# fudan-zvg/PARTNER

Hardware: AMD Instinct MI355X
Metric: frames/sec polar voxelize+PFN+BEV+head, 30k-pt sweep (whole job) (higher is better)
Workload: dtype f32

## Files before the change

### partner_amd/csrc/conv_wchain.hip

```cpp
#include "pn_common.h"
#include "wino_planes.h"
#include <algorithm>
#include <cstdlib>

namespace {

using f32x16 = __attribute__((ext_vector_type(16))) float;
using f32x4 = __attribute__((ext_vector_type(4))) float;
using f32x2 = __attribute__((ext_vector_type(2))) float;

struct WChainArgs {
  const float* vin;
  const float* w;
  const float* scale;
  const float* shift;
  float* vout;
  float* out;
  int B, H, W, Wq, Cin, Cout;
  int wq_log2;
  int out_ps, out_co;
  long long out_img, out_row;
  int act;
  int total_quads;
  int qtiles, ctiles;
// ... 304 lines not shown
    if (!(PN_WCHAIN_EXP & 2) || first) {
#pragma unroll
      for (int r = 0; r < 4; ++r) d[slot][r] = __builtin_bit_cast(f32x4, __builtin_amdgcn_raw_buffer_load_b128(rsrc_v, voff, so_v + (unsigned)r * row16, 0));
    }
    if (!(PN_WCHAIN_EXP & 4) || first) {
#pragma unroll
      for (int s2 = 0; s2 < 4; ++s2) u[slot][s2] = __builtin_bit_cast(f32x4, __builtin_amdgcn_raw_buffer_load_b128(rsrc_w, uoff, so_u + (unsigned)(s2 * 48) * cp16, 0));
    }
  };
  first = true;
  load_step(cg0, 0);
  __builtin_amdgcn_sched_barrier(0);
  load_step(cg0 + 1, 1);
  __builtin_amdgcn_sched_barrier(0);
  first = false;
  WC_STAMP(1);
  for (int cg = cg0; cg <= cg_last; cg += 2) {
#pragma unroll
    for (int slot = 0; slot < 2; ++slot) {
      const int nx = cg + 2 + slot <= cg_last ? cg + 2 + slot : cg_last;
      f32x4 b[4];
      if constexpr (PN_WCHAIN_EXP & 1) {
        b[0] = d[slot][0]; b[1] = d[slot][1]; b[2] = d[slot][2]; b[3] = d[slot][3];
      } else {
#pragma unroll
        for (int e = 0; e < 4; e += 2) {
          f32x2 x0 = {d[slot][0][e], d[slot][0][e + 1]}, x1 = {d[slot][1][e], d[slot][1][e + 1]}, x2 = {d[slot][2][e], d[slot][2][e + 1]},
                x3 = {d[slot][3][e], d[slot][3][e + 1]};
          f32x2 r0, r1, r2, r3;
          asm volatile("v_pk_add_f32 %0, %4, %6 neg_lo:[0,1] neg_hi:[0,1]\n\t"
                       "v_pk_add_f32 %1, %5, %6\n\t"
                       "v_pk_add_f32 %2, %6, %5 neg_lo:[0,1] neg_hi:[0,1]\n\t"
                       "v_pk_add_f32 %3, %5, %7 neg_lo:[0,1] neg_hi:[0,1]"
                       : "=&v"(r0), "=&v"(r1), "=&v"(r2), "=&v"(r3)
                       : "v"(x0), "v"(x1), "v"(x2), "v"(x3));
          b[0][e] = r0[0]; b[0][e + 1] = r0[1];
          b[1][e] = r1[0]; b[1][e + 1] = r1[1];
          b[2][e] = r2[0]; b[2][e + 1] = r2[1];
          b[3][e] = r3[0]; b[3][e + 1] = r3[1];
        }
      }
      if constexpr (PN_WCHAIN_EXP & 8) __builtin_amdgcn_s_setprio(2);
#pragma unroll
      for (int j = 0; j < 4; ++j)
#pragma unroll
        for (int s2 = 0; s2 < 4; ++s2) acc[s2] = __builtin_amdgcn_mfma_f32_32x32x2f32(u[slot][s2][j], b[s2][j], acc[s2], 0, 0, 0);
      if constexpr (PN_WCHAIN_EXP & 8) __builtin_amdgcn_s_setprio(0);
      __builtin_amdgcn_sched_barrier(0);
      load_step(nx, slot);
      __builtin_amdgcn_sched_barrier(0);
    }
  }
  WC_STAMP(2);
  if (bid != bid0) __syncthreads();
#pragma unroll
  for (int g = 0; g < 4; ++g) {
    f32x4 r0, r1;
#pragma unroll
    for (int k = 0; k < 4; ++k) {
      const int r = 4 * g + k;
      r0[k] = (acc[0][r] + acc[1][r]) + acc[2][r];
      r1[k] = (acc[1][r] - acc[2][r]) - acc[3][r];
    }
    J[((w * 2 + 0) * 4 + g) * 64 + lane] = r0;
    J[((w * 2 + 1) * 4 + g) * 64 + lane] = r1;
  }
  __syncthreads();
  for (int vw = w; vw < CT * 8; vw += NW) {
    const int ect = vw >> 3, g = (vw >> 1) & 3, row = vw & 1;
    const int c0 = (ctile * CT + ect) * 32 + 8 * g + 4 * lh;
    wchain_finish<QT>(
        a, c0, li, lh, lo,
        [&](int q, int b) {
          f32x4 m = J[(((q + 6 * (KS * (ect + CT * b))) * 2 + row) * 4 + g) * 64 + lane];
#pragma unroll
          for (int k = 1; k < KS; ++k) m += J[(((q + 6 * (k + KS * (ect + CT * b))) * 2 + row) * 4 + g) * 64 + lane];
          return m;
        },
        [&](int b, int& img, int& r, int& xq) {
          int t;
          wchain_coords(img0, t0, Hh, a.wq_log2, 32 * b + li, img, t, xq);
          r = 2 * t + row;
        },
        a.st_part ? a.st_part + ((size_t)qt * 2 + row) * a.Cout * 2 : nullptr, a.strata_rows > 0 ? ((2 * t0) / a.strata_rows) * a.Cout : 0);
  }
  WC_STAMP(3);
  }
}

template <int KS, int CT, int QT>
__global__ __launch_bounds__(64 * 6 * KS * CT * QT) void conv_wchain2_kernel(WChainArgs a) {
  wchain2_body<KS, CT, QT>(a, blockIdx.x, gridDim.x);
}

template <int SH>
__device__ __forceinline__ void wchain3_kloop(const WChainArgs& a, const __amdgpu_buffer_rsrc_t rsrc_v, const __amdgpu_buffer_rsrc_t rsrc_w, const int p,
                                              const unsigned voff, const unsigned uoff, f32x16 (&acc)[3]) {
  const unsigned cp16 = (unsigned)a.cout_pad * 16u;
  const unsigned row16 = (unsigned)a.Wq * 16u;
  f32x4 d[2][5], u[2][3];
  bool first = false;
  auto load_step = [&](int cg, int slot) __attribute__((always_inline)) {
    const unsigned so_v = (unsigned)((p * a.cg_in + cg) * 2) * a.plane_bytes + (unsigned)SH * row16;
    const unsigned so_u = (unsigned)((((cg >> 2) * 6 + 3 * SH) * 6 + p) * 8 + (cg & 3) * 2) * cp16;
    if (!(PN_WCHAIN_EXP & 2) || first) {
#pragma unroll
      for (int r = 0; r < 5; ++r) d[slot][r] = __builtin_bit_cast(f32x4, __builtin_amdgcn_raw_buffer_load_b128(rsrc_v, voff, so_v + (unsigned)r * row16, 0));
    }
    if (!(PN_WCHAIN_EXP & 4) || first) {
#pragma unroll
      for (int s2 = 0; s2 < 3; ++s2) u[slot][s2] = __builtin_bit_cast(f32x4, __builtin_amdgcn_raw_buffer_load_b128(rsrc_w, uoff, so_u + (unsigned)(s2 * 48) * cp16, 0));
    }
  };
  const int cg_last = a.cg_in - 1;
  first = true;
  load_step(0, 0);
  __builtin_amdgcn_sched_barrier(0);
  load_step(1, 1);
  __builtin_amdgcn_sched_barrier(0);
  first = false;
  for (int cg = 0; cg <= cg_last; cg += 2) {
#pragma unroll
    for (int slot = 0; slot < 2; ++slot) {
      const int nx = cg + 2 + slot <= cg_last ? cg + 2 + slot : cg_last;
      f32x4 b[3];
      const f32x4 c4 = {4.f, 4.f, 4.f, 4.f}, m4 = {-4.f, -4.f, -4.f, -4.f}, m5 = {-5.f, -5.f, -5.f, -5.f}, c2 = {2.f, 2.f, 2.f, 2.f}, m2 = {-2.f, -2.f, -2.f, -2.f};
      if constexpr (PN_WCHAIN_EXP & 1) {
        b[0] = d[slot][0]; b[1] = d[slot][1]; b[2] = d[slot][2];
      } else if constexpr (SH == 0) {
        const f32x4 e = __builtin_elementwise_fma(m4, d[slot][2], d[slot][4]), o = __builtin_elementwise_fma(m4, d[slot][1], d[slot][3]);
        b[0] = __builtin_elementwise_fma(c4, d[slot][0], __builtin_elementwise_fma(m5, d[slot][2], d[slot][4]));
        b[1] = e + o;
        b[2] = e - o;
      } else {
        const f32x4 f = d[slot][3] - d[slot][1], t = d[slot][2] - d[slot][0];
        b[0] = __builtin_elementwise_fma(c2, t, f);
        b[1] = __builtin_elementwise_fma(m2, t, f);
        b[2] = __builtin_elementwise_fma(c4, d[slot][0], __builtin_elementwise_fma(m5, d[slot][2], d[slot][4]));
      }
#pragma unroll
      for (int j = 0; j < 4; ++j)
#pragma unroll
        for (int s2 = 0; s2 < 3; ++s2) {
          if (PN_WC3_EXP & 1) acc[s2][0] += u[slot][s2][j] * b[s2][j];
          else acc[s2] = __builtin_amdgcn_mfma_f32_32x32x2f32(u[slot][s2][j], b[s2][j], acc[s2], 0, 0, 0);
        }
      __builtin_amdgcn_sched_barrier(0);
      load_step(nx, slot);
      __builtin_amdgcn_sched_barrier(0);
    }
  }
}

template <int QT>
__global__ __launch_bounds__(64 * 12) void conv_wchain3_kernel(WChainArgs a) {
  constexpr int NW = 12;
  extern __shared__ __attribute__((aligned(16))) float smem[];
  WCHAIN_FETCH_ARGS(a);
  const int tid = threadIdx.x, lane = tid & 63;
  const int w = __builtin_amdgcn_readfirstlane(tid >> 6);
  const int p = w % 6, sh = w / 6;
  const int li = lane & 31, lh = lane >> 5;
  const __amdgpu_buffer_rsrc_t rsrc_v = __builtin_amdgcn_make_buffer_rsrc(const_cast<float*>(a.vin), 0, a.vin_bytes, 0x00020000);
  const __amdgpu_buffer_rsrc_t rsrc_w = __builtin_amdgcn_make_buffer_rsrc(const_cast<float*>(a.w), 0, a.w_bytes, 0x00020000);
  const int Hq = a.H >> 2;
  f32x4* J = reinterpret_cast<f32x4*>(smem);
  f32x4* carry = J + 6 * 4 * 4 * 64;
  const float lo = a.act == PN_ACT_RELU ? 0.f : -__builtin_inff();
  const int bid = blockIdx.x;
  int qt, ctile;
  if ((a.qtiles & 7) == 0) {
    const int xcd = bid & 7, slot = bid >> 3;
    qt = xcd * (a.qtiles >> 3) + slot / a.ctiles;
    ctile = slot - (slot / a.ctiles) * a.ctiles;
  } else {
    qt = bid / a.ctiles;
    ctile = bid - qt * a.ctiles;
  }
  const int n0 = ctile * 32;
  const int o0 = qt * 32 * QT;
  const int rg0 = o0 >> a.wq_log2, img0 = rg0 / Hq, t0 = rg0 - img0 * Hq;
  const unsigned uoff = (unsigned)(((size_t)lh * a.cout_pad + n0 + li) * 16);
#pragma unroll 1
  for (int sub = 0; sub < QT; ++sub) {
    int img, t, xq;
    wchain_coords(img0, t0, Hq, a.wq_log2, 32 * sub + li, img, t, xq);
    const unsigned voff = (unsigned)(((img * (a.H + 2) + 4 * t) * a.Wq + xq) * 16) + (unsigned)lh * a.plane_bytes;
    f32x16 acc[3];
#pragma unroll
    for (int s = 0; s < 3; ++s)
#pragma unroll
      for (int r = 0; r < 16; ++r) acc[s][r] = 0.f;
    if (sh == 0) wchain3_kloop<0>(a, rsrc_v, rsrc_w, p, voff, uoff, acc);
    else wchain3_kloop<1>(a, rsrc_v, rsrc_w, p, voff, uoff, acc);
    if (PN_WC3_EXP & 2) {
      if (acc[0][0] + acc[1][3] + acc[2][7] == 1234.5f) J[lane] = f32x4{acc[0][1], acc[1][1], acc[2][1], 0.f};
    }
    if (sub > 0) __syncthreads();
    if (sh == 0 && !(PN_WC3_EXP & 2)) {
#pragma unroll
      for (int g = 0; g < 4; ++g) {
        f32x4 r0, r1, r2;
#pragma unroll
        for (int k = 0; k < 4; ++k) {
          const int r = 4 * g + k;
          r0[k] = (acc[0][r] + acc[1][r]) + acc[2][r];
          r1[k] = acc[1][r] - acc[2][r];
          r2[k] = acc[1][r] + acc[2][r];
        }
        J[((p * 4 + 0) * 4 + g) * 64 + lane] = r0;
        J[((p * 4 + 1) * 4 + g) * 64 + lane] = r1;
        J[((p * 4 + 2) * 4 + g) * 64 + lane] = r2;
        J[((p * 4 + 3) * 4 + g) * 64 + lane] = r1;
      }
    }
    __syncthreads();
    if (sh == 1 && !(PN_WC3_EXP & 2)) {
#pragma unroll
      for (int g = 0; g < 4; ++g) {
        f32x4 r0, r1, r2, r3;
#pragma unroll
        for (int k = 0; k < 4; ++k) {
          const int r = 4 * g + k;
          const float s34 = acc[0][r] + acc[1][r], d34 = acc[0][r] - acc[1][r];
          r0[k] = s34;
          r1[k] = 2.f * d34;
          r2[k] = 4.f * s34;
          r3[k] = 8.f * d34 + acc[2][r];
        }
        J[((p * 4 + 0) * 4 + g) * 64 + lane] += r0;
        J[((p * 4 + 1) * 4 + g) * 64 + lane] += r1;
        J[((p * 4 + 2) * 4 + g) * 64 + lane] += r2;
        J[((p * 4 + 3) * 4 + g) * 64 + lane] += r3;
      }
    }
    __syncthreads();
    for (int vw = w; vw < ((PN_WC3_EXP & 4) ? 0 : 16); vw += NW) {
      const int g = vw >> 2, row = vw & 3;
      const int c0 = ctile * 32 + 8 * g + 4 * lh;
      if constexpr (QT == 1) {
        wchain_finish<1>(
            a, c0, li, lh, lo, [&](int q, int) { return J[((q * 4 + row) * 4 + g) * 64 + lane]; },
            [&](int, int& im, int& r, int& x) { im = img; r = 4 * t + row; x = xq; });
      } else {
        f32x4 sc = {1.f, 1.f, 1.f, 1.f}, shf = {0.f, 0.f, 0.f, 0.f};
        if (a.scale) sc = *reinterpret_cast<const f32x4*>(a.scale + c0);
        if (a.shift) shf = *reinterpret_cast<const f32x4*>(a.shift + c0);
        f32x4 m[6], y[4];
#pragma unroll
        for (int q = 0; q < 6; ++q) m[q] = J[((q * 4 + row) * 4 + g) * 64 + lane];
        {
          const f32x4 s12 = m[1] + m[2], d12 = m[1] - m[2], s34 = m[3] + m[4], d34 = m[3] - m[4];
          const f32x4 lo4 = {lo, lo, lo, lo};
          y[0] = __builtin_elementwise_max(__builtin_elementwise_fma((m[0] + s12) + s34, sc, shf), lo4);
          y[1] = __builtin_elementwise_max(__builtin_elementwise_fma(d12 + 2.f * d34, sc, shf), lo4);
          y[2] = __builtin_elementwise_max(__builtin_elementwise_fma(s12 + 4.f * s34, sc, shf), lo4);
          y[3] = __builtin_elementwise_max(__builtin_elementwise_fma((d12 + 8.f * d34) + m[5], sc, shf), lo4);
        }
        const int r = 4 * t + row;
        if (a.out) {
          float* o = a.out + (size_t)img * a.out_img + (size_t)r * a.out_row + (size_t)(4 * xq) * a.out_ps + a.out_co + c0;
#pragma unroll
          for (int px = 0; px < 4; ++px) *reinterpret_cast<f32x4*>(o + (size_t)px * a.out_ps) = y[px];
        }
        if (a.vout) {
          f32x4* cr = carry + ((row * 4 + g) * 2 + lh) * 5;
          f32x4 l, rr;
#pragma unroll
          for (int j = 0; j < 4; ++j) {
            l[j] = __shfl_up(y[3][j], 1, 32);
            rr[j] = __shfl_down(y[0][j], 1, 32);
          }
          const f32x4 z4 = {0.f, 0.f, 0.f, 0.f};
          auto store_planes = [&](const f32x4 (&d)[6], int xs) {
            f32x4 vv[6];
            wchain_input_transform(d, vv);
            float* o = a.vout + ((size_t)(c0 >> 3) * 2 + lh) * (a.plane_bytes >> 2) + ((size_t)(img * (a.H + 2) + r + 1) * a.Wq + xs) * 4;
            const size_t pstride = (size_t)a.cg_out * 2 * (a.plane_bytes >> 2);
#pragma unroll
            for (int q = 0; q < 6; ++q) *reinterpret_cast<f32x4*>(o + q * pstride) = vv[q];
            if (r == 0) {
#pragma unroll
              for (int q = 0; q < 6; ++q) *reinterpret_cast<f32x4*>(o + q * pstride - (size_t)a.Wq * 4) = z4;
            }
            if (r == a.H - 1) {
#pragma unroll
              for (int q = 0; q < 6; ++q) *reinterpret_cast<f32x4*>(o + q * pstride + (size_t)a.Wq * 4) = z4;
            }
          };
          if (sub == 0) {
            if (li == 31) {
              cr[0] = y[0]; cr[1] = y[1]; cr[2] = y[2]; cr[3] = y[3]; cr[4] = l;
            } else {
              f32x4 d[6];
              d[0] = xq > 0 ? l : z4;
              d[1] = y[0]; d[2] = y[1]; d[3] = y[2]; d[4] = y[3];
              d[5] = rr;
              store_planes(d, xq);
            }
          } else {
            if (li == 0) {
              f32x4 d[6];
              d[0] = cr[4]; d[1] = cr[0]; d[2] = cr[1]; d[3] = cr[2]; d[4] = cr[3];
              d[5] = y[0];
              store_planes(d, xq - 1);
              l = cr[3];
            }
            f32x4 d[6];
            d[0] = l;
            d[1] = y[0]; d[2] = y[1]; d[3] = y[2]; d[4] = y[3];
            d[5] = xq + 1 < a.Wq ? rr : z4;
            store_planes(d, xq);
          }
        }
      }
    }
  }
}

__global__ void pack_wino44_weight_kernel(const float* __restrict__ w, int cout, int cin, int cout_pad, float* __restrict__ packed, size_t total) {
  for (size_t i = blockIdx.x * (size_t)blockDim.x + threadIdx.x; i < total; i += (size_t)gridDim.x * blockDim.x) {
    size_t r = i;
    const int k1 = r & 3; r >>= 2;
    const int n = (int)(r % cout_pad); r /= cout_pad;
    const int k4 = r & 7; r >>= 3;
    const int q = (int)(r % 6); r /= 6;
    const int s = (int)(r % 6);
    const int chunk = (int)(r / 6);
    const int c = chunk * 32 + k4 * 4 + k1;
    double v = 0.0;
    if (n < cout && c < cin) {
      const float* g = w + ((size_t)n * cin + c) * 9;
      auto fold = [](int pos, double g0, double g1, double g2) {
        return pos == 0 ? g0 / 4.0 : pos == 1 ? -(g0 + g1 + g2) / 6.0 : pos == 2 ? -(g0 - g1 + g2) / 6.0 : pos == 3 ? g0 / 24.0 + g1 / 12.0 + g2 / 6.0
               : pos == 4 ? g0 / 24.0 - g1 / 12.0 + g2 / 6.0 : g2;
      };
      double row[3];
      for (int kw = 0; kw < 3; ++kw) row[kw] = fold(s, g[kw], g[3 + kw], g[6 + kw]);
      v = fold(q, row[0], row[1], row[2]);
    }
    packed[i] = (float)v;
  }
}

constexpr int kChainMultiJobs = 4;
struct WChainMulti {
  int njobs;
  int first[kChainMultiJobs + 1];
  WChainArgs job[kChainMultiJobs];
};

template <int KS, int CT, int QT>
__global__ __launch_bounds__(64 * 6 * KS * CT * QT) void conv_wchain2_multi_kernel(WChainMulti by_value) {
  typedef const __attribute__((address_space(4))) int* kptr_t;
  const kptr_t base = (kptr_t)__builtin_amdgcn_kernarg_segment_ptr();
  const int njobs = base[offsetof(WChainMulti, njobs) / 4];
  const int t = blockIdx.x;
  int j = 0;
  for (int k = 1; k < njobs; ++k)
    if (t >= base[offsetof(WChainMulti, first) / 4 + k]) j = k;
  j = __builtin_amdgcn_readfirstlane(j);
  const int local = t - base[offsetof(WChainMulti, first) / 4 + j];
  constexpr int JW = sizeof(WChainArgs) / 4;
  union { WChainArgs a; int w[JW]; } u;
  const kptr_t src = base + offsetof(WChainMulti, job) / 4 + j * JW;
#pragma unroll
  for (int i = 0; i < JW; ++i) u.w[i] = src[i];
  wchain2_body<KS, CT, QT>(u.a, local, 1 << 30);
}

__global__ void pack_wino24_weight_kernel(const float* __restrict__ w, int cout, int cin, int cout_pad, float* __restrict__ packed, size_t total) {
  for (size_t i = blockIdx.x * (size_t)blockDim.x + threadIdx.x; i < total; i += (size_t)gridDim.x * blockDim.x) {
    size_t r = i;
    const int k1 = r & 3; r >>= 2;
    const int n = (int)(r % cout_pad); r /= cout_pad;
    const int k4 = r & 7; r >>= 3;
    const int q = (int)(r % 6); r /= 6;
    const int s = (int)(r & 3);
    const int chunk = (int)(r >> 2);
    const int c = chunk * 32 + k4 * 4 + k1;
    double v = 0.0;
    if (n < cout && c < cin) {
      const float* g = w + ((size_t)n * cin + c) * 9;
      double row[3];
      for (int kw = 0; kw < 3; ++kw) {
        const double g0 = g[kw], g1 = g[3 + kw], g2 = g[6 + kw];
        row[kw] = s == 0 ? g0 : s == 1 ? (g0 + g1 + g2) * 0.5 : s == 2 ? (g0 - g1 + g2) * 0.5 : g2;
      }
      const double g0 = row[0], g1 = row[1], g2 = row[2];
      v = q == 0 ? g0 / 4.0 : q == 1 ? -(g0 + g1 + g2) / 6.0 : q == 2 ? -(g0 - g1 + g2) / 6.0 : q == 3 ? g0 / 24.0 + g1 / 12.0 + g2 / 6.0
          : q == 4 ? g0 / 24.0 - g1 / 12.0 + g2 / 6.0 : g2;
    }
    packed[i] = (float)v;
  }
}

__global__ __launch_bounds__(256) void wchain_v_from_nhwc_kernel(const float* __restrict__ in, float* __restrict__ vout, int B, int H, int W, int Wq, int C,
                                                                 long long in_img, long long in_row, int in_ps, int in_co, int total_quads,
                                                                 unsigned plane_floats) {
  const int c4n = C >> 2;
  for (long long it = blockIdx.x * (long long)blockDim.x + threadIdx.x; it < (long long)total_quads * c4n; it += (long long)gridDim.x * blockDim.x) {
    const int c4 = (int)(it / total_quads);
    const int Q = (int)(it - (long long)c4 * total_quads);
    const int rowi = Q / Wq, xq = Q - rowi * Wq;
    const int img = rowi / H, r = rowi - img * H;
    const float* px = in + (size_t)img * in_img + (size_t)r * in_row + (size_t)(4 * xq) * in_ps + in_co + c4 * 4;
    f32x4 d[6], v[6];
    const f32x4 z = {0.f, 0.f, 0.f, 0.f};
    d[0] = xq > 0 ? *reinterpret_cast<const f32x4*>(px - in_ps) : z;
#pragma unroll
    for (int k = 0; k < 4; ++k) d[1 + k] = *reinterpret_cast<const f32x4*>(px + (size_t)k * in_ps);
    d[5] = xq + 1 < Wq ? *reinterpret_cast<const f32x4*>(px + (size_t)4 * in_ps) : z;
    wchain_input_transform(d, v);
    float* o = vout + (size_t)c4 * plane_floats + ((size_t)(img * (H + 2) + r + 1) * Wq + xq) * 4;
    const size_t pstride = (size_t)c4n * plane_floats;
#pragma unroll
    for (int q = 0; q < 6; ++q) *reinterpret_cast<f32x4*>(o + q * pstride) = v[q];
    if (r == 0) {
#pragma unroll
      for (int q = 0; q < 6; ++q) *reinterpret_cast<f32x4*>(o + q * pstride - (size_t)Wq * 4) = z;
    }
    if (r == H - 1) {
#pragma unroll
      for (int q = 0; q < 6; ++q) *reinterpret_cast<f32x4*>(o + q * pstride + (size_t)Wq * 4) = z;
    }
  }
}

constexpr int kHeadFinJobs = 8;
struct HeadFinJob {
  const float* part;
  int cout_total, c_off, cmid;
  int strata;
  const float* gamma;
  const float* beta;
  float eps;
  float* tab;
};
struct HeadFinArgs {
  int njobs, B, rows, tile_rows;
  long long row_pixels;
  HeadFinJob job[kHeadFinJobs];
};

__global__ __launch_bounds__(256) void wchain_head_finalize_kernel(HeadFinArgs f) {
  __shared__ double red[2][4];
  const int S0 = 8;
  const int j = blockIdx.x / (f.B * S0), rem = blockIdx.x - j * (f.B * S0), b = rem / S0, s = rem - b * S0;
  if (j >= f.njobs) return;
  const HeadFinJob& jb = f.job[j];
  const int S = jb.strata > 1 ? jb.strata : 1;
  if (s >= S) return;
  const int tid = threadIdx.x;
  const int tiles_b = f.rows / f.tile_rows;
  const float2* part = reinterpret_cast<const float2*>(jb.part);
  if (S == 1) {
    __shared__ double sl1[4][64], sl2[4][64];
    for (int c0 = 0; c0 < jb.cmid; c0 += 64) {
      const int c = c0 + (tid & 63), slice = tid >> 6;
      double a1 = 0.0, a2 = 0.0;
      if (c < jb.cmid) {
#pragma unroll 8
        for (int e = slice; e < tiles_b * 2; e += 4) {
          const float2 v = part[((size_t)b * tiles_b * 2 + e) * jb.cout_total + jb.c_off + c];
          a1 += (double)v.x;
          a2 += (double)v.y;
        }
      }
      __syncthreads();
      sl1[slice][tid & 63] = a1;
      sl2[slice][tid & 63] = a2;
      __syncthreads();
      if (tid < 64 && c < jb.cmid) {
        const double t1 = ((sl1[0][tid] + sl1[1][tid]) + sl1[2][tid]) + sl1[3][tid], t2 = ((sl2[0][tid] + sl2[1][tid]) + sl2[2][tid]) + sl2[3][tid];
        const double n = (double)f.rows * (double)f.row_pixels;
        const double mean = t1 / n;
        double var = t2 / n - mean * mean;
        var = var < 0.0 ? 0.0 : var;
        const float rstd = (float)(1.0 / sqrt(var + (double)jb.eps));
        const float ga = jb.gamma ? jb.gamma[c] : 1.f, be = jb.beta ? jb.beta[c] : 0.f;
        const float A = ga * rstd;
        reinterpret_cast<float2*>(jb.tab)[(size_t)b * jb.cmid + c] = make_float2(A, be - (float)mean * A);
      }
    }
    return;
  }
  const int tiles_s = tiles_b / S;
  const int count = tiles_s * 2 * jb.cmid;
  double t1 = 0.0, t2 = 0.0;
  for (int e = tid; e < count; e += 256) {
    const int ent = e / jb.cmid, c = e - ent * jb.cmid;
    const float2 v = part[((size_t)(b * tiles_b + s * tiles_s) * 2 + ent) * jb.cout_total + jb.c_off + c];
    t1 += (double)v.x;
    t2 += (double)v.y;
  }
  t1 = pn::wave_sum(t1);
  t2 = pn::wave_sum(t2);
  if ((tid & 63) == 0) {
    red[0][tid >> 6] = t1;
    red[1][tid >> 6] = t2;
  }
  __syncthreads();
  const double u1 = ((red[0][0] + red[0][1]) + red[0][2]) + red[0][3], u2 = ((red[1][0] + red[1][1]) + red[1][2]) + red[1][3];
  const double n = (double)(f.rows / S) * (double)f.row_pixels * jb.cmid;
  const double mean = u1 / n;
  double var = u2 / n - mean * mean;
  var = var < 0.0 ? 0.0 : var;
  const float fmean = (float)mean, rstd = (float)(1.0 / sqrt(var + (double)jb.eps));
  for (int c = tid; c < jb.cmid; c += 256) {
    const float ga = jb.gamma ? jb.gamma[s * jb.cmid + c] : 1.f, be = jb.beta ? jb.beta[s * jb.cmid + c] : 0.f;
    const float A = ga * rstd;
    reinterpret_cast<float2*>(jb.tab)[((size_t)b * S + s) * jb.cmid + c] = make_float2(A, be - fmean * A);
  }
}

static int chain_grid_limit() {
  static const int force = [] { const char* e = getenv("PN_WCHAIN_GRID"); return e ? atoi(e) : -1; }();
  if (force == 0) return 1 << 30;
  if (force > 0) return force;
  static int cus[64] = {0};
  int dev = 0;
  (void)hipGetDevice(&dev);
  if (dev < 0 || dev >= 64) return 256;
  if (cus[dev] == 0) {
    int n = 0;
    cus[dev] = (hipDeviceGetAttribute(&n, hipDeviceAttributeMultiprocessorCount, dev) == hipSuccess && n >= 8) ? n / 8 * 8 : 256;
  }
  return cus[dev];
}

struct ChainForm { int na, nb, ks, ct; };

static inline int frame_h(const pn_conv_desc* d) { return d->transpose_hw ? d->in_w : d->in_h; }
static inline int frame_w(const pn_conv_desc* d) { return d->transpose_hw ? d->in_h : d->in_w; }

static bool chain_form(const pn_conv_desc* d, ChainForm& f) {
  const int fh = frame_h(d), fw = frame_w(d);
  if (fw % 4) return false;
  const int wq = fw / 4;
  if (wq & (wq - 1)) return false;
  const long long quads = (long long)d->batch * fh * wq;
  static const int force = [] { const char* e = getenv("PN_WCHAIN_FORM"); return e ? atoi(e) : 0; }();
  const ChainForm cands[] = {{2, 2, 1, 2}, {1, 2, 2, 1}, {1, 1, 2, 1}};
  int idx = 0;
  for (const ChainForm& c : cands) {
    ++idx;
    if (force && force != idx) continue;
    const int tq = 32 * c.nb, tc = 32 * c.na * c.ct;
    if (tq % wq != 0 || quads % tq != 0 || d->cout % tc != 0 || (d->cin / 8) % c.ks != 0 || tq / wq > fh) continue;
    const long long blocks = quads / tq * (d->cout / tc);
    if (!force && blocks < 192 && idx < 3) continue;
    f = c;
    return true;
  }
  return false;
}

template <int NA, int NB, int KS, int CT>
static void launch_chain(const WChainArgs& a, hipStream_t st, bool prof, const pn::ProfileSlot& ps) {
  constexpr int NW = 6 * KS * CT;
  constexpr size_t smem = (size_t)NW * NB * 4 * 64 * 16;
  static bool done[64] = {false};
  if (pn::first_use_on_device(done))
    (void)hipFuncSetAttribute(reinterpret_cast<const void*>(&conv_wchain_kernel<NA, NB, KS, CT>), hipFuncAttributeMaxDynamicSharedMemorySize, (int)smem);
  const dim3 grid((unsigned)std::min(a.qtiles * a.ctiles, chain_grid_limit()));
  if (prof) hipExtLaunchKernelGGL((conv_wchain_kernel<NA, NB, KS, CT>), grid, dim3(64 * NW), smem, st, ps.start, ps.stop, 0, a);
  else hipLaunchKernelGGL((conv_wchain_kernel<NA, NB, KS, CT>), grid, dim3(64 * NW), smem, st, a);
}

struct Chain2Form { int ks, ct, qt; };

static bool chain2_form(const pn_conv_desc* d, Chain2Form& f, bool head = false) {
  const int fh = frame_h(d), fw = frame_w(d);
  if (fw % 4 || fh % 2) return false;
  const int wq = fw / 4;
  if (wq & (wq - 1)) return false;
  const long long octs = (long long)d->batch * (fh / 2) * wq;
  static const int prefer = [] { const char* e = getenv("PN_WCHAIN2_PREFER"); return e ? atoi(e) : 1; }();
  const bool wide_first = !head && (prefer == 2 || (prefer == 1 && d->frames_in_flight > 1)) && (octs / 64) * (d->cout / 32) >= 128;
  const Chain2Form cands_a[] = {{2, 1, 1}, {1, 1, 2}}, cands_b[] = {{1, 1, 2}, {2, 1, 1}};
  const Chain2Form* cands = wide_first ? cands_b : cands_a;
  for (int ci = 0; ci < 2; ++ci) {
    const Chain2Form& c = cands[ci];
    const int tq = 32 * c.qt, tc = 32 * c.ct;
    if (tq % wq != 0 || octs % tq != 0 || d->cout % tc != 0 || (d->cin / 8) % (2 * c.ks) != 0 || tq / wq > fh / 2) continue;
    f = c;
    return true;
  }
  return false;
}

template <int KS, int CT, int QT>
static void launch_chain2(const WChainArgs& a, hipStream_t st, bool prof, const pn::ProfileSlot& ps) {
  constexpr int NW = 6 * KS * CT * QT;
  constexpr size_t smem = (size_t)NW * 2 * 4 * 64 * 16;
  static bool done[64] = {false};
  if (pn::first_use_on_device(done))
    (void)hipFuncSetAttribute(reinterpret_cast<const void*>(&conv_wchain2_kernel<KS, CT, QT>), hipFuncAttributeMaxDynamicSharedMemorySize, (int)smem);
  const dim3 grid((unsigned)std::min(a.qtiles * a.ctiles, chain_grid_limit()));
  if (prof) hipExtLaunchKernelGGL((conv_wchain2_kernel<KS, CT, QT>), grid, dim3(64 * NW), smem, st, ps.start, ps.stop, 0, a);
  else hipLaunchKernelGGL((conv_wchain2_kernel<KS, CT, QT>), grid, dim3(64 * NW), smem, st, a);
}

template <int KS, int CT, int QT>
static void launch_chain2_multi(const WChainMulti& m, hipStream_t st, bool prof, const pn::ProfileSlot& ps) {
  constexpr int NW = 6 * KS * CT * QT;
  constexpr size_t smem = (size_t)NW * 2 * 4 * 64 * 16;
  static bool done[64] = {false};
  if (pn::first_use_on_device(done))
    (void)hipFuncSetAttribute(reinterpret_cast<const void*>(&conv_wchain2_multi_kernel<KS, CT, QT>), hipFuncAttributeMaxDynamicSharedMemorySize, (int)smem);
  const dim3 grid((unsigned)m.first[m.njobs]);
  if (prof) hipExtLaunchKernelGGL((conv_wchain2_multi_kernel<KS, CT, QT>), grid, dim3(64 * NW), smem, st, ps.start, ps.stop, 0, m);
  else hipLaunchKernelGGL((conv_wchain2_multi_kernel<KS, CT, QT>), grid, dim3(64 * NW), smem, st, m);
}

}

extern "C" {

size_t pn_wino4_planes_floats(int batch, int h, int w, int c) {
  if (batch < 1 || h < 1 || w < 4 || w % 4 || c < 8 || c % 8) return 0;
  return (size_t)6 * c * batch * (h + 2) * (w / 4);
}

static int chain_basic_ok(const pn_conv_desc* d, bool allow_strata);

int pn_conv_wino4_chain_supported(const pn_conv_desc* d) {
  if (!chain_basic_ok(d, false)) return 0;
  ChainForm f;
  return chain_form(d, f) ? 1 : 0;
}

static int chain_basic_ok(const pn_conv_desc* d, bool allow_strata) {
  if (!d) return 0;
  if (!(d->kh == 3 && d->kw == 3 && d->stride == 1 && d->pad_h == 1 && d->pad_w == 1 && d->groups == 1 && !d->deconv2x2 &&
        (d->range_strata <= 1 || allow_strata) && !d->accumulate && d->pad_h_end == 0 && d->pad_w_end == 0))
    return 0;
  if (d->batch < 1 || frame_h(d) < 1 || frame_w(d) < 4 || d->cin % 32 || d->cout % 32 || d->cin < 32) return 0;
  if (!(d->act == PN_ACT_NONE || d->act == PN_ACT_RELU)) return 0;
  if ((unsigned long long)pn_wino4_planes_floats(d->batch, frame_h(d), frame_w(d), std::max(d->cin, d->cout)) * 4ull >= (1ull << 32)) return 0;
  return 1;
}

int pn_wino4_planes_from_nhwc_f32(const float* in, int batch, int h, int w, int c, int in_pixel_stride, int in_channel_offset, int transpose_hw,
                                  float* planes, pn_stream_t stream) {
  const int stored_w = w;
  if (transpose_hw) std::swap(h, w);
  PN_REQUIRE(in && planes && pn_wino4_planes_floats(batch, h, w, c) > 0, "wino4_planes_from_nhwc: bad arguments");
  PN_REQUIRE(in_pixel_stride % 4 == 0 && in_channel_offset % 4 == 0 && in_pixel_stride >= in_channel_offset + c && ((uintptr_t)in & 15) == 0 &&
                 ((uintptr_t)planes & 15) == 0,
             "wino4_planes_from_nhwc: strides / offsets must be multiples of 4 floats, pointers 16-byte aligned");
  const int wq = w / 4;
  const long long quads = (long long)batch * h * wq;
  PN_REQUIRE(quads < (1ll << 30), "wino4_planes_from_nhwc: map too large");
  const unsigned plane_floats = (unsigned)((size_t)batch * (h + 2) * wq * 4);
  const long long items = quads * (c / 4);
  const long long in_img = (long long)h * w * in_pixel_stride;
  const long long in_row = transpose_hw ? in_pixel_stride : (long long)stored_w * in_pixel_stride;
  const int in_px = transpose_hw ? stored_w * in_pixel_stride : in_pixel_stride;
  hipLaunchKernelGGL(wchain_v_from_nhwc_kernel, dim3((unsigned)std::min<long long>(8192, (items + 255) / 256)), dim3(256), 0, pn::S(stream), in, planes, batch, h,
                     w, wq, c, in_img, in_row, in_px, in_channel_offset, (int)quads, plane_floats);
  return pn::check_launch("wchain_v_from_nhwc_kernel");
}

int pn_conv2d_wino4_chain_f32(const pn_conv_desc* d, const float* planes_in, const float* packed_w, const float* scale, const float* shift,
                              float* planes_out, float* out_nhwc, pn_stream_t stream) {
  PN_REQUIRE(d && planes_in && packed_w && (planes_out || out_nhwc), "conv_wino4_chain: null pointer");
  PN_REQUIRE(pn_conv_wino4_chain_supported(d), "conv_wino4_chain: layer shape not supported (3x3 / stride 1 / pad 1, cin and cout multiples of 32, "
                                               "row-aligned tiles)");
  PN_REQUIRE(((uintptr_t)planes_in & 15) == 0 && ((uintptr_t)packed_w & 15) == 0 && ((uintptr_t)planes_out & 15) == 0 && ((uintptr_t)out_nhwc & 15) == 0 &&
                 ((uintptr_t)scale & 15) == 0 && ((uintptr_t)shift & 15) == 0,
             "conv_wino4_chain: pointers must be 16-byte aligned");
  if (out_nhwc)
    PN_REQUIRE(d->out_pixel_stride >= d->out_channel_offset + d->cout && d->out_pixel_stride % 4 == 0 && d->out_channel_offset % 4 == 0 &&
                   (unsigned long long)d->batch * d->in_h * d->in_w * d->out_pixel_stride < (1ull << 40),
               "conv_wino4_chain: output channel slice must fit the pixel stride, in multiples of 4 floats");
  ChainForm f;
  chain_form(d, f);
  WChainArgs a{};
  a.vin = planes_in; a.w = packed_w; a.scale = scale; a.shift = shift; a.vout = planes_out; a.out = out_nhwc;
  a.B = d->batch; a.H = frame_h(d); a.W = frame_w(d); a.Wq = a.W / 4; a.Cin = d->cin; a.Cout = d->cout;
  a.out_co = d->out_channel_offset;
  a.out_img = (long long)d->in_h * d->in_w * d->out_pixel_stride;
  a.out_ps = d->transpose_hw ? d->in_w * d->out_pixel_stride : d->out_pixel_stride;
  a.out_row = d->transpose_hw ? d->out_pixel_stride : (long long)d->in_w * d->out_pixel_stride;
  a.wq_log2 = __builtin_ctz((unsigned)a.Wq);
  a.act = d->act;
  a.total_quads = d->batch * a.H * a.Wq;
  a.qtiles = a.total_quads / (32 * f.nb);
  a.ctiles = d->cout / (32 * f.na * f.ct);
  a.cg_in = d->cin / 8; a.cg_out = d->cout / 8;
  a.cout_pad = pn::cdiv(d->cout, 128) * 128;
  a.plane_bytes = (unsigned)((size_t)d->batch * (a.H + 2) * a.Wq * 16);
  a.vin_bytes = (unsigned)(pn_wino4_planes_floats(d->batch, a.H, a.W, d->cin) * 4);
  a.w_bytes = (unsigned)(pn_conv_wino4_packed_weight_floats(d->cout, d->cin) * 4);
#ifdef PN_WCHAIN_STAMP
  a.stamps = pn_wchain_stamp_buffer;
#endif
  pn::ProfileSlot ps{};
  const bool prof = pn::take_profile_slot(ps);
  hipStream_t st = pn::S(stream);
  if (f.na == 2 && f.nb == 2 && f.ks == 1 && f.ct == 2) launch_chain<2, 2, 1, 2>(a, st, prof, ps);
  else if (f.na == 1 && f.nb == 2 && f.ks == 2 && f.ct == 1) launch_chain<1, 2, 2, 1>(a, st, prof, ps);
  else launch_chain<1, 1, 2, 1>(a, st, prof, ps);
  return pn::check_launch("conv_wchain_kernel");
}

size_t pn_conv_wino24_packed_weight_floats(int cout, int cin) {
  return (size_t)pn::cdiv(cin, 32) * 4 * 6 * 8 * (size_t)(pn::cdiv(cout, 128) * 128) * 4;
}

int pn_pack_conv_weight_wino24_f32(const float* w_oihw, int cout, int cin, float* packed, pn_stream_t stream) {
  PN_REQUIRE(w_oihw && packed && cout >= 1 && cin >= 1, "pack_conv_weight_wino24: bad arguments");
  const size_t total = pn_conv_wino24_packed_weight_floats(cout, cin);
  hipLaunchKernelGGL(pack_wino24_weight_kernel, dim3((unsigned)std::min<size_t>(4096, (total + 255) / 256)), dim3(256), 0, pn::S(stream), w_oihw, cout, cin,
                     pn::cdiv(cout, 128) * 128, packed, total);
  return pn::check_launch("pack_wino24_weight_kernel");
}

static int chain2_ok(const pn_conv_desc* d, bool head, Chain2Form& f) {
  if (!chain_basic_ok(d, head) || !chain2_form(d, f, head)) return 0;
  if (d->range_strata > 1) {
    if (!d->transpose_hw || frame_h(d) % d->range_strata) return 0;
    const int rows = frame_h(d) / d->range_strata, tile_rows = 2 * (32 * f.qt) / (frame_w(d) / 4);
    if (rows % tile_rows) return 0;
  }
  return 1;
}

int pn_conv_wino24_chain_supported(const pn_conv_desc* d) {
  Chain2Form f;
  return chain2_ok(d, false, f);
}

static int chain2_fill(const pn_conv_desc* d, const float* planes_in, const float* packed_w24, const float* scale, const float* shift, float* planes_out,
                       float* out_nhwc, float* stat_partials, bool head, WChainArgs& a, Chain2Form& f) {
  PN_REQUIRE(d && planes_in && packed_w24 && (planes_out || out_nhwc), "conv_wino24_chain: null pointer");
  PN_REQUIRE(chain2_ok(d, head, f), "conv_wino24_chain: layer shape not supported (3x3 / stride 1 / pad 1, even height, cin and cout multiples of 32, "
                                    "row-pair-aligned tiles; range strata: transposed map, whole tiles per stratum)");
  PN_REQUIRE(((uintptr_t)planes_in & 15) == 0 && ((uintptr_t)packed_w24 & 15) == 0 && ((uintptr_t)planes_out & 15) == 0 && ((uintptr_t)out_nhwc & 15) == 0 &&
                 ((uintptr_t)scale & 15) == 0 && ((uintptr_t)shift & 15) == 0 && ((uintptr_t)stat_partials & 7) == 0,
             "conv_wino24_chain: pointers must be 16-byte aligned");
  PN_REQUIRE(!stat_partials || d->act == PN_ACT_NONE, "conv_wino24_chain: statistics are those of the stored output (no activation)");
  if (out_nhwc)
    PN_REQUIRE(d->out_pixel_stride >= d->out_channel_offset + d->cout && d->out_pixel_stride % 4 == 0 && d->out_channel_offset % 4 == 0,
               "conv_wino24_chain: output channel slice must fit the pixel stride, in multiples of 4 floats");
  a = WChainArgs{};
  a.vin = planes_in; a.w = packed_w24; a.scale = scale; a.shift = shift; a.vout = planes_out; a.out = out_nhwc;
  a.B = d->batch; a.H = frame_h(d); a.W = frame_w(d); a.Wq = a.W / 4; a.Cin = d->cin; a.Cout = d->cout;
  a.out_co = d->out_channel_offset;
  a.out_img = (long long)d->in_h * d->in_w * d->out_pixel_stride;
  a.out_ps = d->transpose_hw ? d->in_w * d->out_pixel_stride : d->out_pixel_stride;
  a.out_row = d->transpose_hw ? d->out_pixel_stride : (long long)d->in_w * d->out_pixel_stride;
  a.wq_log2 = __builtin_ctz((unsigned)a.Wq);
  a.act = d->act;
  a.total_quads = d->batch * a.H * a.Wq;
  a.qtiles = (a.total_quads / 2) / (32 * f.qt);
  a.ctiles = d->cout / (32 * f.ct);
  a.cg_in = d->cin / 8; a.cg_out = d->cout / 8;
  a.cout_pad = pn::cdiv(d->cout, 128) * 128;
  a.plane_bytes = (unsigned)((size_t)d->batch * (a.H + 2) * a.Wq * 16);
  a.vin_bytes = (unsigned)(pn_wino4_planes_floats(d->batch, a.H, a.W, d->cin) * 4);
  const int sets = d->range_strata > 1 ? d->range_strata : 1;
  a.w_stratum_bytes = (unsigned)(pn_conv_wino24_packed_weight_floats(d->cout, d->cin) * 4);
  a.w_bytes = a.w_stratum_bytes * (unsigned)sets;
  a.strata_rows = sets > 1 ? a.H / sets : 0;
  a.st_part = stat_partials;
#ifdef PN_WCHAIN_STAMP
  a.stamps = pn_wchain_stamp_buffer;
#endif
  return PN_OK;
}

static int chain2_run(const pn_conv_desc* d, const float* planes_in, const float* packed_w24, const float* scale, const float* shift, float* planes_out,
                      float* out_nhwc, float* stat_partials, bool head, pn_stream_t stream) {
  WChainArgs a;
  Chain2Form f;
  const int rc = chain2_fill(d, planes_in, packed_w24, scale, shift, planes_out, out_nhwc, stat_partials, head, a, f);
  if (rc != PN_OK) return rc;
  pn::ProfileSlot ps{};
  const bool prof = pn::take_profile_slot(ps);
  hipStream_t st = pn::S(stream);
  if (f.ks == 2) launch_chain2<2, 1, 1>(a, st, prof, ps);
  else launch_chain2<1, 1, 2>(a, st, prof, ps);
  return pn::check_launch("conv_wchain2_kernel");
}

int pn_conv2d_wino24_chain_f32(const pn_conv_desc* d, const float* planes_in, const float* packed_w24, const float* scale, const float* shift,
                               float* planes_out, float* out_nhwc, pn_stream_t stream) {
  return chain2_run(d, planes_in, packed_w24, scale, shift, planes_out, out_nhwc, nullptr, false, stream);
}

size_t pn_conv_wino44_packed_weight_floats(int cout, int cin) {
  return (size_t)pn::cdiv(cin, 32) * 6 * 6 * 8 * (size_t)(pn::cdiv(cout, 128) * 128) * 4;
}

int pn_pack_conv_weight_wino44_f32(const float* w_oihw, int cout, int cin, float* packed, pn_stream_t stream) {
  PN_REQUIRE(w_oihw && packed && cout >= 1 && cin >= 1, "pack_conv_weight_wino44: bad arguments");
  const size_t total = pn_conv_wino44_packed_weight_floats(cout, cin);
  hipLaunchKernelGGL(pack_wino44_weight_kernel, dim3((unsigned)std::min<size_t>(4096, (total + 255) / 256)), dim3(256), 0, pn::S(stream), w_oihw, cout, cin,
                     pn::cdiv(cout, 128) * 128, packed, total);
  return pn::check_launch("pack_wino44_weight_kernel");
}

int pn_conv_wino44_chain_supported(const pn_conv_desc* d) {
  if (!chain_basic_ok(d, false) || d->range_strata > 1) return 0;
  const int fh = frame_h(d), fw = frame_w(d);
  if (fw % 4 || fh % 4) return 0;
  const int wq = fw / 4;
  if ((wq & (wq - 1)) || wq > 64) return 0;
  const int tq = wq == 64 ? 64 : 32;
  const long long hexes = (long long)d->batch * (fh / 4) * wq;
  if (tq % wq || hexes % tq || tq / wq > fh / 4 || (d->cin / 8) % 2) return 0;
  return 1;
}

int pn_conv2d_wino44_chain_f32(const pn_conv_desc* d, const float* planes_in, const float* packed_w44, const float* scale, const float* shift,
                               float* planes_out, float* out_nhwc, pn_stream_t stream) {
  PN_REQUIRE(d && planes_in && packed_w44 && (planes_out || out_nhwc), "conv_wino44_chain: null pointer");
  PN_REQUIRE(pn_conv_wino44_chain_supported(d), "conv_wino44_chain: layer shape not supported (3x3 / stride 1 / pad 1, height a multiple of 4, at most 32 quads "
                                                "per row, cin and cout multiples of 32)");
  PN_REQUIRE(((uintptr_t)planes_in & 15) == 0 && ((uintptr_t)packed_w44 & 15) == 0 && ((uintptr_t)planes_out & 15) == 0 && ((uintptr_t)out_nhwc & 15) == 0 &&
                 ((uintptr_t)scale & 15) == 0 && ((uintptr_t)shift & 15) == 0,
             "conv_wino44_chain: pointers must be 16-byte aligned");
  if (out_nhwc)
    PN_REQUIRE(d->out_pixel_stride >= d->out_channel_offset + d->cout && d->out_pixel_stride % 4 == 0 && d->out_channel_offset % 4 == 0,
               "conv_wino44_chain: output channel slice must fit the pixel stride, in multiples of 4 floats");
  WChainArgs a{};
  a.vin = planes_in; a.w = packed_w44; a.scale = scale; a.shift = shift; a.vout = planes_out; a.out = out_nhwc;
  a.B = d->batch; a.H = frame_h(d); a.W = frame_w(d); a.Wq = a.W / 4; a.Cin = d->cin; a.Cout = d->cout;
  a.out_co = d->out_channel_offset;
  a.out_img = (long long)d->in_h * d->in_w * d->out_pixel_stride;
  a.out_ps = d->transpose_hw ? d->in_w * d->out_pixel_stride : d->out_pixel_stride;
  a.out_row = d->transpose_hw ? d->out_pixel_stride : (long long)d->in_w * d->out_pixel_stride;
  a.wq_log2 = __builtin_ctz((unsigned)a.Wq);
  a.act = d->act;
  a.total_quads = d->batch * a.H * a.Wq;
  const int qt2 = a.Wq == 64 ? 2 : 1;
  a.qtiles = (a.total_quads / 4) / (32 * qt2);
  a.ctiles = d->cout / 32;
  a.cg_in = d->cin / 8; a.cg_out = d->cout / 8;
  a.cout_pad = pn::cdiv(d->cout, 128) * 128;
  a.plane_bytes = (unsigned)((size_t)d->batch * (a.H + 2) * a.Wq * 16);
  a.vin_bytes = (unsigned)(pn_wino4_planes_floats(d->batch, a.H, a.W, d->cin) * 4);
  a.w_bytes = (unsigned)(pn_conv_wino44_packed_weight_floats(d->cout, d->cin) * 4);
#ifdef PN_WCHAIN_STAMP
  a.stamps = pn_wchain_stamp_buffer;
#endif
  constexpr size_t smem = (size_t)6 * 4 * 4 * 64 * 16 + (size_t)4 * 4 * 2 * 5 * 16;
  static bool done[64] = {false};
  if (pn::first_use_on_device(done)) {
    (void)hipFuncSetAttribute(reinterpret_cast<const void*>(&conv_wchain3_kernel<1>), hipFuncAttributeMaxDynamicSharedMemorySize, (int)smem);
    (void)hipFuncSetAttribute(reinterpret_cast<const void*>(&conv_wchain3_kernel<2>), hipFuncAttributeMaxDynamicSharedMemorySize, (int)smem);
  }
  pn::ProfileSlot ps{};
  const bool prof = pn::take_profile_slot(ps);
  const dim3 grid((unsigned)(a.qtiles * a.ctiles));
  if (qt2 == 2) {
    if (prof) hipExtLaunchKernelGGL(conv_wchain3_kernel<2>, grid, dim3(64 * 12), smem, pn::S(stream), ps.start, ps.stop, 0, a);
    else hipLaunchKernelGGL(conv_wchain3_kernel<2>, grid, dim3(64 * 12), smem, pn::S(stream), a);
  } else {
    if (prof) hipExtLaunchKernelGGL(conv_wchain3_kernel<1>, grid, dim3(64 * 12), smem, pn::S(stream), ps.start, ps.stop, 0, a);
    else hipLaunchKernelGGL(conv_wchain3_kernel<1>, grid, dim3(64 * 12), smem, pn::S(stream), a);
  }
  return pn::check_launch("conv_wchain3_kernel");
}

size_t pn_conv_wino24_chain_stat_floats(const pn_conv_desc* d) {
  Chain2Form f;
  if (!chain2_ok(d, true, f)) return 0;
  const long long octs = (long long)d->batch * (frame_h(d) / 2) * (frame_w(d) / 4);
  return (size_t)(octs / (32 * f.qt)) * 2 * d->cout * 2;
}

int pn_conv_wino24_chain_stat_tile_rows(const pn_conv_desc* d) {
  Chain2Form f;
  if (!chain2_ok(d, true, f)) return 0;
  return 2 * (32 * f.qt) / (frame_w(d) / 4);
}

int pn_conv2d_wino24_chain_head_f32(const pn_conv_desc* d, const float* planes_in, const float* packed_w24, const float* scale, const float* shift,
                                    float* planes_out, float* out_nhwc, float* stat_partials, pn_stream_t stream) {
  return chain2_run(d, planes_in, packed_w24, scale, shift, planes_out, out_nhwc, stat_partials, true, stream);
}

int pn_conv2d_wino24_chain_head_multi_f32(const pn_chain_head_job* jobs, int njobs, pn_stream_t stream) {
  PN_REQUIRE(jobs && njobs >= 1 && njobs <= kChainMultiJobs, "conv_wino24_chain_head_multi: 1 - 4 jobs");
  WChainMulti m{};
  m.njobs = njobs;
  Chain2Form f0{};
  for (int j = 0; j < njobs; ++j) {
    const pn_chain_head_job& q = jobs[j];
    Chain2Form f;
    const int rc = chain2_fill(q.desc, q.planes_in, q.packed_w24, q.scale, q.shift, q.planes_out, q.out_nhwc, q.stat_partials, true, m.job[j], f);
    if (rc != PN_OK) return rc;
    if (j == 0) f0 = f;
    PN_REQUIRE(f.ks == f0.ks && f.ct == f0.ct && f.qt == f0.qt, "conv_wino24_chain_head_multi: the jobs must share one kernel form (same map, same cin)");
    m.first[j + 1] = m.first[j] + m.job[j].qtiles * m.job[j].ctiles;
  }
  pn::ProfileSlot ps{};
  const bool prof = pn::take_profile_slot(ps);
  hipStream_t st = pn::S(stream);
  static const int ks1 = [] { const char* e = getenv("PN_WCHAIN_MULTI_KS1"); return e ? atoi(e) : 1; }();
  const bool others = ks1 == 2 || (ks1 == 1 && jobs[0].desc->frames_in_flight > 1);
  if (f0.ks == 2 && others && m.job[0].cg_in <= 8 && m.first[njobs] >= 2 * chain_grid_limit()) launch_chain2_multi<1, 1, 1>(m, st, prof, ps);
  else if (f0.ks == 2) launch_chain2_multi<2, 1, 1>(m, st, prof, ps);
  else launch_chain2_multi<1, 1, 2>(m, st, prof, ps);
  return pn::check_launch("conv_wchain2_multi_kernel");
}

int pn_wino24_chain_head_finalize_f32(const pn_head_stat_job* jobs, int njobs, int batch, int frame_rows, int frame_row_pixels, int tile_rows,
                                      pn_stream_t stream) {
  PN_REQUIRE(jobs && njobs >= 1 && njobs <= kHeadFinJobs && batch >= 1 && frame_rows >= 1 && tile_rows >= 1 && frame_rows % tile_rows == 0,
             "wino24_chain_head_finalize: bad arguments");
  HeadFinArgs f{};
  f.njobs = njobs; f.B = batch; f.rows = frame_rows; f.tile_rows = tile_rows; f.row_pixels = frame_row_pixels;
  for (int j = 0; j < njobs; ++j) {
    const pn_head_stat_job& q = jobs[j];
    PN_REQUIRE(q.partials && q.table && q.channels >= 1 && q.channel_offset >= 0 && q.channel_offset + q.channels <= q.cout_total,
               "wino24_chain_head_finalize: bad job");
    PN_REQUIRE(q.strata <= 8 && (q.strata <= 1 ? q.channels <= 256 : (frame_rows / tile_rows) % q.strata == 0),
               "wino24_chain_head_finalize: per-channel jobs take <= 256 channels; strata (<= 8) must divide the sample's tiles");
    f.job[j] = HeadFinJob{q.partials, q.cout_total, q.channel_offset, q.channels, q.strata, q.gamma, q.beta, q.eps, q.table};
  }
  hipLaunchKernelGGL(wchain_head_finalize_kernel, dim3((unsigned)(njobs * batch * 8)), dim3(256), 0, pn::S(stream), f);
  return pn::check_launch("wchain_head_finalize_kernel");
}

}
```

Before: 1766.

## Compute two output-channel tiles per block in wino44 chain conv to reuse input

Adds a two-column variant of the Winograd 4x4 chain kernel in which each block accumulates two 32-channel output tiles. Each loaded and transformed input tile then feeds both sets of MFMAs, which halves input-plane loads and input transforms per output channel. The variant is chosen automatically when cout is a multiple of 64 and the grid stays large enough, and an env var can force either variant. In exchange the block doubles its accumulator registers, adds extra syncs for the serialized epilogue, uses more carry LDS, and launches fewer blocks.

```diff
diff --git a/partner_amd/csrc/conv_wchain.hip b/partner_amd/csrc/conv_wchain.hip
--- a/partner_amd/csrc/conv_wchain.hip
+++ b/partner_amd/csrc/conv_wchain.hip
@@ -480,7 +480,73 @@
   }
 }
 
-template <int QT>
+template <int SH>
+__device__ __forceinline__ void wchain3_kloop2(const WChainArgs& a, const __amdgpu_buffer_rsrc_t rsrc_v, const __amdgpu_buffer_rsrc_t rsrc_w, const int p,
+                                               const unsigned voff, const unsigned uoff, f32x16 (&acc)[2][3]) {
+  const unsigned cp16 = (unsigned)a.cout_pad * 16u;
+  const unsigned row16 = (unsigned)a.Wq * 16u;
+  f32x4 d[5], u[2][3];
+  bool first = false;
+  auto load_d = [&](int cg) __attribute__((always_inline)) {
+    const unsigned so_v = (unsigned)((p * a.cg_in + cg) * 2) * a.plane_bytes + (unsigned)SH * row16;
+    if (!(PN_WCHAIN_EXP & 2) || first) {
+#pragma unroll
+      for (int r = 0; r < 5; ++r) d[r] = __builtin_bit_cast(f32x4, __builtin_amdgcn_raw_buffer_load_b128(rsrc_v, voff, so_v + (unsigned)r * row16, 0));
+    }
+  };
+  auto load_u = [&](int cg, int c) __attribute__((always_inline)) {
+    const unsigned so_u = (unsigned)((((cg >> 2) * 6 + 3 * SH) * 6 + p) * 8 + (cg & 3) * 2) * cp16 + (unsigned)c * 512u;
+    if (!(PN_WCHAIN_EXP & 4) || first) {
+#pragma unroll
+      for (int s2 = 0; s2 < 3; ++s2) u[c][s2] = __builtin_bit_cast(f32x4, __builtin_amdgcn_raw_buffer_load_b128(rsrc_w, uoff, so_u + (unsigned)(s2 * 48) * cp16, 0));
+    }
+  };
+  const int cg_last = a.cg_in - 1;
+  first = true;
+  load_d(0);
+  __builtin_amdgcn_sched_barrier(0);
+  load_u(0, 0);
+  __builtin_amdgcn_sched_barrier(0);
+  load_u(0, 1);
+  __builtin_amdgcn_sched_barrier(0);
+  first = false;
+  for (int cg = 0; cg <= cg_last; ++cg) {
+    const int nx = cg < cg_last ? cg + 1 : cg_last;
+    f32x4 b[3];
+    const f32x4 c4 = {4.f, 4.f, 4.f, 4.f}, m4 = {-4.f, -4.f, -4.f, -4.f}, m5 = {-5.f, -5.f, -5.f, -5.f}, c2 = {2.f, 2.f, 2.f, 2.f}, m2 = {-2.f, -2.f, -2.f, -2.f};
+    if constexpr (PN_WCHAIN_EXP & 1) {
+      b[0] = d[0]; b[1] = d[1]; b[2] = d[2];
+    } else if constexpr (SH == 0) {
+      const f32x4 e = __builtin_elementwise_fma(m4, d[2], d[4]), o = __builtin_elementwise_fma(m4, d[1], d[3]);
+      b[0] = __builtin_elementwise_fma(c4, d[0], __builtin_elementwise_fma(m5, d[2], d[4]));
+      b[1] = e + o;
+      b[2] = e - o;
+    } else {
+      const f32x4 f = d[3] - d[1], t = d[2] - d[0];
+      b[0] = __builtin_elementwise_fma(c2, t, f);
+      b[1] = __builtin_elementwise_fma(m2, t, f);
+      b[2] = __builtin_elementwise_fma(c4, d[0], __builtin_elementwise_fma(m5, d[2], d[4]));
+    }
+    __builtin_amdgcn_sched_barrier(0);
+    load_d(nx);
+    __builtin_amdgcn_sched_barrier(0);
+#pragma unroll
+    for (int c = 0; c < 2; ++c) {
+#pragma unroll
+      for (int j = 0; j < 4; ++j)
+#pragma unroll
+        for (int s2 = 0; s2 < 3; ++s2) {
+          if (PN_WC3_EXP & 1) acc[c][s2][0] += u[c][s2][j] * b[s2][j];
+          else acc[c][s2] = __builtin_amdgcn_mfma_f32_32x32x2f32(u[c][s2][j], b[s2][j], acc[c][s2], 0, 0, 0);
+        }
+      __builtin_amdgcn_sched_barrier(0);
+      load_u(nx, c);
+      __builtin_amdgcn_sched_barrier(0);
+    }
+  }
+}
+
+template <int QT, int NC>
 __global__ __launch_bounds__(64 * 12) void conv_wchain3_kernel(WChainArgs a) {
   constexpr int NW = 12;
   extern __shared__ __attribute__((aligned(16))) float smem[];
@@ -505,26 +571,43 @@
     qt = bid / a.ctiles;
     ctile = bid - qt * a.ctiles;
   }
-  const int n0 = ctile * 32;
+  const int n0 = ctile * 32 * NC;
   const int o0 = qt * 32 * QT;
   const int rg0 = o0 >> a.wq_log2, img0 = rg0 / Hq, t0 = rg0 - img0 * Hq;
   const unsigned uoff = (unsigned)(((size_t)lh * a.cout_pad + n0 + li) * 16);
 #pragma unroll 1
   for (int sub = 0; sub < QT; ++sub) {
-    int img, t, xq;
-    wchain_coords(img0, t0, Hq, a.wq_log2, 32 * sub + li, img, t, xq);
+    int li, lh, img, t, xq;
+    auto lane_coords = [&]() __attribute__((always_inline)) {
+      int ln = lane;
+      if constexpr (NC == 2) asm volatile("" : "+v"(ln));
+      li = ln & 31;
+      lh = ln >> 5;
+      wchain_coords(img0, t0, Hq, a.wq_log2, 32 * sub + li, img, t, xq);
+    };
+    lane_coords();
     const unsigned voff = (unsigned)(((img * (a.H + 2) + 4 * t) * a.Wq + xq) * 16) + (unsigned)lh * a.plane_bytes;
-    f32x16 acc[3];
-#pragma unroll
-    for (int s = 0; s < 3; ++s)
-#pragma unroll
-      for (int r = 0; r < 16; ++r) acc[s][r] = 0.f;
-    if (sh == 0) wchain3_kloop<0>(a, rsrc_v, rsrc_w, p, voff, uoff, acc);
-    else wchain3_kloop<1>(a, rsrc_v, rsrc_w, p, voff, uoff, acc);
+    f32x16 acc[NC][3];
+#pragma unroll
+    for (int c = 0; c < NC; ++c)
+#pragma unroll
+      for (int s = 0; s < 3; ++s)
+#pragma unroll
+        for (int r = 0; r < 16; ++r) acc[c][s][r] = 0.f;
+    if constexpr (NC == 1) {
+      if (sh == 0) wchain3_kloop<0>(a, rsrc_v, rsrc_w, p, voff, uoff, acc[0]);
+      else wchain3_kloop<1>(a, rsrc_v, rsrc_w, p, voff, uoff, acc[0]);
+    } else {
+      if (sh == 0) wchain3_kloop2<0>(a, rsrc_v, rsrc_w, p, voff, uoff, acc);
+      else wchain3_kloop2<1>(a, rsrc_v, rsrc_w, p, voff, uoff, acc);
+      lane_coords();
+    }
+#pragma unroll
+    for (int c = 0; c < NC; ++c) {
     if (PN_WC3_EXP & 2) {
-      if (acc[0][0] + acc[1][3] + acc[2][7] == 1234.5f) J[lane] = f32x4{acc[0][1], acc[1][1], acc[2][1], 0.f};
-    }
-    if (sub > 0) __syncthreads();
+      if (acc[c][0][0] + acc[c][1][3] + acc[c][2][7] == 1234.5f) J[lane] = f32x4{acc[c][0][1], acc[c][1][1], acc[c][2][1], 0.f};
+    }
+    if (sub > 0 || c > 0) __syncthreads();
     if (sh == 0 && !(PN_WC3_EXP & 2)) {
 #pragma unroll
       for (int g = 0; g < 4; ++g) {
@@ -532,9 +615,9 @@
 #pragma unroll
         for (int k = 0; k < 4; ++k) {
           const int r = 4 * g + k;
-          r0[k] = (acc[0][r] + acc[1][r]) + acc[2][r];
-          r1[k] = acc[1][r] - acc[2][r];
-          r2[k] = acc[1][r] + acc[2][r];
+          r0[k] = (acc[c][0][r] + acc[c][1][r]) + acc[c][2][r];
+          r1[k] = acc[c][1][r] - acc[c][2][r];
+          r2[k] = acc[c][1][r] + acc[c][2][r];
         }
         J[((p * 4 + 0) * 4 + g) * 64 + lane] = r0;
         J[((p * 4 + 1) * 4 + g) * 64 + lane] = r1;
@@ -550,11 +633,11 @@
 #pragma unroll
         for (int k = 0; k < 4; ++k) {
           const int r = 4 * g + k;
-          const float s34 = acc[0][r] + acc[1][r], d34 = acc[0][r] - acc[1][r];
+          const float s34 = acc[c][0][r] + acc[c][1][r], d34 = acc[c][0][r] - acc[c][1][r];
           r0[k] = s34;
           r1[k] = 2.f * d34;
           r2[k] = 4.f * s34;
-          r3[k] = 8.f * d34 + acc[2][r];
+          r3[k] = 8.f * d34 + acc[c][2][r];
         }
         J[((p * 4 + 0) * 4 + g) * 64 + lane] += r0;
         J[((p * 4 + 1) * 4 + g) * 64 + lane] += r1;
@@ -565,7 +648,7 @@
     __syncthreads();
     for (int vw = w; vw < ((PN_WC3_EXP & 4) ? 0 : 16); vw += NW) {
       const int g = vw >> 2, row = vw & 3;
-      const int c0 = ctile * 32 + 8 * g + 4 * lh;
+      const int c0 = (ctile * NC + c) * 32 + 8 * g + 4 * lh;
       if constexpr (QT == 1) {
         wchain_finish<1>(
             a, c0, li, lh, lo, [&](int q, int) { return J[((q * 4 + row) * 4 + g) * 64 + lane]; },
@@ -592,7 +675,7 @@
           for (int px = 0; px < 4; ++px) *reinterpret_cast<f32x4*>(o + (size_t)px * a.out_ps) = y[px];
         }
         if (a.vout) {
-          f32x4* cr = carry + ((row * 4 + g) * 2 + lh) * 5;
+          f32x4* cr = carry + (((c * 4 + row) * 4 + g) * 2 + lh) * 5;
           f32x4 l, rr;
 #pragma unroll
           for (int j = 0; j < 4; ++j) {
@@ -642,6 +725,7 @@
           }
         }
       }
+    }
     }
   }
 }
@@ -940,6 +1024,23 @@
   const dim3 grid((unsigned)m.first[m.njobs]);
   if (prof) hipExtLaunchKernelGGL((conv_wchain2_multi_kernel<KS, CT, QT>), grid, dim3(64 * NW), smem, st, ps.start, ps.stop, 0, m);
   else hipLaunchKernelGGL((conv_wchain2_multi_kernel<KS, CT, QT>), grid, dim3(64 * NW), smem, st, m);
+}
+
+static int wino44_cols(int cout, int qtiles) {
+  static const int force = [] { const char* e = getenv("PN_WCHAIN3_COLS"); return e ? atoi(e) : 0; }();
+  if (cout % 64) return 1;
+  if (force == 1 || force == 2) return force;
+  return (long long)qtiles * (cout / 64) >= 128 ? 2 : 1;
+}
+
+template <int QT, int NC>
+static void launch_chain3(const WChainArgs& a, dim3 grid, hipStream_t st, bool prof, const pn::ProfileSlot& ps) {
+  constexpr size_t smem = (size_t)6 * 4 * 4 * 64 * 16 + (size_t)NC * 4 * 4 * 2 * 5 * 16;
+  static bool done[64] = {false};
+  if (pn::first_use_on_device(done))
+    (void)hipFuncSetAttribute(reinterpret_cast<const void*>(&conv_wchain3_kernel<QT, NC>), hipFuncAttributeMaxDynamicSharedMemorySize, (int)smem);
+  if (prof) hipExtLaunchKernelGGL((conv_wchain3_kernel<QT, NC>), grid, dim3(64 * 12), smem, st, ps.start, ps.stop, 0, a);
+  else hipLaunchKernelGGL((conv_wchain3_kernel<QT, NC>), grid, dim3(64 * 12), smem, st, a);
 }
 
 }
@@ -1166,7 +1267,8 @@
   a.total_quads = d->batch * a.H * a.Wq;
   const int qt2 = a.Wq == 64 ? 2 : 1;
   a.qtiles = (a.total_quads / 4) / (32 * qt2);
-  a.ctiles = d->cout / 32;
+  const int nc = wino44_cols(d->cout, a.qtiles);
+  a.ctiles = d->cout / (32 * nc);
   a.cg_in = d->cin / 8; a.cg_out = d->cout / 8;
   a.cout_pad = pn::cdiv(d->cout, 128) * 128;
   a.plane_bytes = (unsigned)((size_t)d->batch * (a.H + 2) * a.Wq * 16);
@@ -1175,21 +1277,16 @@
 #ifdef PN_WCHAIN_STAMP
   a.stamps = pn_wchain_stamp_buffer;
 #endif
-  constexpr size_t smem = (size_t)6 * 4 * 4 * 64 * 16 + (size_t)4 * 4 * 2 * 5 * 16;
-  static bool done[64] = {false};
-  if (pn::first_use_on_device(done)) {
-    (void)hipFuncSetAttribute(reinterpret_cast<const void*>(&conv_wchain3_kernel<1>), hipFuncAttributeMaxDynamicSharedMemorySize, (int)smem);
-    (void)hipFuncSetAttribute(reinterpret_cast<const void*>(&conv_wchain3_kernel<2>), hipFuncAttributeMaxDynamicSharedMemorySize, (int)smem);
-  }
   pn::ProfileSlot ps{};
   const bool prof = pn::take_profile_slot(ps);
   const dim3 grid((unsigned)(a.qtiles * a.ctiles));
+  hipStream_t st = pn::S(stream);
   if (qt2 == 2) {
-    if (prof) hipExtLaunchKernelGGL(conv_wchain3_kernel<2>, grid, dim3(64 * 12), smem, pn::S(stream), ps.start, ps.stop, 0, a);
-    else hipLaunchKernelGGL(conv_wchain3_kernel<2>, grid, dim3(64 * 12), smem, pn::S(stream), a);
+    if (nc == 2) launch_chain3<2, 2>(a, grid, st, prof, ps);
+    else launch_chain3<2, 1>(a, grid, st, prof, ps);
   } else {
-    if (prof) hipExtLaunchKernelGGL(conv_wchain3_kernel<1>, grid, dim3(64 * 12), smem, pn::S(stream), ps.start, ps.stop, 0, a);
-    else hipLaunchKernelGGL(conv_wchain3_kernel<1>, grid, dim3(64 * 12), smem, pn::S(stream), a);
+    if (nc == 2) launch_chain3<1, 2>(a, grid, st, prof, ps);
+    else launch_chain3<1, 1>(a, grid, st, prof, ps);
   }
   return pn::check_launch("conv_wchain3_kernel");
 }
```

New measurement: 1860 (median of 6 runs). 1.05x the previous value.
